# y00njaekim/CMU-11785-IDL-1.58bit-ASR

Hardware: AMD Instinct MI355X
Metric: mel-frames/sec (Conformer-S 1.58-bit train step) (higher is better)
Workload: dtype fp32; 1 GPU; conformer-s-1.58bit-train-step; global_batch=32, execution=hip-graph, per_gpu_batch=32, frames=1000, d_model=144, blocks=16, d_ff=576, heads=4, vocab=5004, parallelism=dp1, passes=teacher 2-bit + student 1-bit + SP, conv_pointwise=fp32 (reference)

## Files before the change

### cmu-11785-idl-1.58bit-asr_amd/csrc/convmod.hip

```cpp
#include <math.h>

#include <cstdlib>

#include "ob_fp.h"
#include "ob_launch.h"

namespace ob {

namespace {

constexpr int kThreads = 256;
constexpr size_t kMaxLds = 160 * 1024;

__device__ __forceinline__ float sigm(float x) { return fast_sigmoid(x); }
__device__ __forceinline__ float swish(float y) { return y * sigm(y); }

template <int KT, int R>
__device__ __forceinline__ void conv_window(const float* __restrict__ tile, int C, int c, int tl0,
                                            const float (&wt)[KT], float (&out)[R]) {
  float win[R + KT - 1];
#pragma unroll
  for (int i = 0; i < R + KT - 1; ++i) win[i] = tile[(tl0 + i) * C + c];
#pragma unroll
  for (int r = 0; r < R; ++r) {
// ... 342 lines not shown
}

__device__ __forceinline__ __amdgpu_buffer_rsrc_t rsrc(const float* base, size_t bytes) {
  return __builtin_amdgcn_make_buffer_rsrc(const_cast<float*>(base), (short)0, (int)bytes,
                                           0x00020000);
}
__device__ __forceinline__ float bload(__amdgpu_buffer_rsrc_t r, int off) {
  return __builtin_bit_cast(float, __builtin_amdgcn_raw_buffer_load_b32(r, off, 0, 0));
}
__device__ __forceinline__ void bstore(__amdgpu_buffer_rsrc_t r, int off, float v) {
  __builtin_amdgcn_raw_buffer_store_b32(__builtin_bit_cast(int, v), r, off, 0, 0);
}
typedef float cm_f32x4 __attribute__((ext_vector_type(4)));
__device__ __forceinline__ cm_f32x4 bload4(__amdgpu_buffer_rsrc_t r, int off) {
  return __builtin_bit_cast(cm_f32x4, __builtin_amdgcn_raw_buffer_load_b128(r, off, 0, 0));
}
constexpr int kLBQ = 4;

constexpr int kTT = 64;

template <int KT, int CG>
__global__ __launch_bounds__(kThreads) void cm_fwd_tile_kernel(
    const float* __restrict__ u, const float* __restrict__ wdw, const float* __restrict__ bdw,
    int T, int C, float* __restrict__ z, float* __restrict__ gout) {
  constexpr int P = KT / 2, W = kTT + KT - 1, NW = W * CG;
  constexpr int CQ = CG / 4, NQ = W * CQ;
  __shared__ __attribute__((aligned(16))) float gs[NW];
  const int t0 = blockIdx.x * kTT, b = blockIdx.y, c0 = blockIdx.z * CG;
  const size_t rb = (size_t)b * T;
  const __amdgpu_buffer_rsrc_t ru = rsrc(u + rb * 2 * C, (size_t)T * 2 * C * 4);
  for (int i0 = 0; i0 < NQ; i0 += kLBQ * kThreads) {
    cm_f32x4 va[kLBQ], vb[kLBQ];
#pragma unroll
    for (int q = 0; q < kLBQ; ++q) {
      const int i = i0 + threadIdx.x + q * kThreads;
      const int tl = i / CQ, cq = i - tl * CQ;
      const int t = t0 - P + tl;
      const int tc = t < 0 ? 0 : (t >= T ? T - 1 : t);
      const int off = 4 * (tc * 2 * C + c0 + 4 * (i < NQ ? cq : 0));
      va[q] = bload4(ru, off);
      vb[q] = bload4(ru, off + 4 * C);
    }
#pragma unroll
    for (int q = 0; q < kLBQ; ++q) {
      const int i = i0 + threadIdx.x + q * kThreads;
      if (i >= NQ) break;
      const int tl = i / CQ, cq = i - tl * CQ;
      const int t = t0 - P + tl;
      const bool in = t >= 0 && t < T;
      cm_f32x4 g4;
#pragma unroll
      for (int k = 0; k < 4; ++k) g4[k] = in ? va[q][k] * sigm(vb[q][k]) : 0.0f;
      *reinterpret_cast<cm_f32x4*>(gs + tl * CG + 4 * cq) = g4;
    }
  }
  __syncthreads();
  constexpr int nrb = kTT / kR;
  for (int it = threadIdx.x; it < CG * nrb; it += kThreads) {
    const int c = it % CG, tl0 = kR * (it / CG);
    if (t0 + tl0 >= T) break;
    float wt[KT], out[kR];
#pragma unroll
    for (int j = 0; j < KT; ++j) wt[j] = wdw[(c0 + c) * KT + j];
    conv_window<KT, kR>(gs, CG, c, tl0, wt, out);
    const float bc = bdw ? bdw[c0 + c] : 0.0f;
#pragma unroll
    for (int r = 0; r < kR; ++r) {
      const int t = t0 + tl0 + r;
      if (t < T) {
        z[(rb + t) * C + c0 + c] = out[r] + bc;
        gout[(rb + t) * C + c0 + c] = gs[(tl0 + r + P) * CG + c];
      }
    }
  }
}

template <int KT, int CG>
__global__ __launch_bounds__(kThreads) void cm_bwd_tile_kernel(
    const float* __restrict__ dv, const float* __restrict__ z, const float* __restrict__ g,
    const float* __restrict__ u, const float* __restrict__ stats, const float* __restrict__ coef,
    const float* __restrict__ gamma, const float* __restrict__ beta,
    const float* __restrict__ wdw, int64_t rows_pp, int T, int C, float* __restrict__ du,
    float* __restrict__ wpart, CmWgradEntry* __restrict__ tslot, CmWgradEntry ent) {
  constexpr int P = KT / 2, W = kTT + KT - 1, NW = W * CG;
  constexpr int CQ = CG / 4, NQ = W * CQ;
  if (tslot && blockIdx.x == 0 && blockIdx.y == 0 && blockIdx.z == 0 && threadIdx.x == 0) *tslot = ent;
  __shared__ __attribute__((aligned(16))) float dzs[NW];
  __shared__ __attribute__((aligned(16))) float gs[NW];
  const int t0 = blockIdx.x * kTT, b = blockIdx.y, c0 = blockIdx.z * CG;
  const size_t rb = (size_t)b * T;
  const int pass = (int)(rb / rows_pp);
  const size_t sl = (size_t)T * C * 4;
  const __amdgpu_buffer_rsrc_t rdv = rsrc(dv + rb * C, sl), rz = rsrc(z + rb * C, sl),
                               rg = rsrc(g + rb * C, sl);
  const __amdgpu_buffer_rsrc_t ru = rsrc(u + rb * 2 * C, 2 * sl), rdu = rsrc(du + rb * 2 * C, 2 * sl);
  for (int i0 = 0; i0 < NQ; i0 += kLBQ * kThreads) {
// ... 254 lines not shown
  cm_wgrad_final_block((int)blockIdx.x, wpart, nblk, C, K, dw, db);
}

__global__ __launch_bounds__(64 * kWfSlices) void cm_wgrad_table_kernel(
    const CmWgradEntry* __restrict__ tab) {
  const CmWgradEntry e = tab[blockIdx.y];
  if ((int)blockIdx.x * 64 >= e.C * (e.K + 1)) return;
  cm_wgrad_final_block((int)blockIdx.x, e.wpart, e.nblk, e.C, e.K, e.dw, e.db);
}

int rows_chunks(int64_t rows_pp, int64_t C) {
  const int64_t per = 8 * (kThreads / (C / 4));
  const int64_t s = (rows_pp + per - 1) / per;
  const int64_t cap = (rows_pp + kSB - 1) / kSB;
  const int64_t m = cap < 512 ? cap : 512;
  return (int)(s < 1 ? 1 : (s > m ? m : s));
}

int stats_chunks(int64_t rows_pp) {
  const int64_t s = (rows_pp + kSB - 1) / kSB;
  return (int)(s < 1 ? 1 : (s > 512 ? 512 : s));
}

size_t lds_fwd(int C, int K, int TT) { return sizeof(float) * ((size_t)(TT + K - 1) * C + (size_t)C * K); }
size_t lds_bwd(int C, int K, int TT) {
  return sizeof(float) * (2 * (size_t)(TT + K - 1) * C + (size_t)C * K);
}

int pick_tt(int64_t C, int64_t K) {
  for (int tt : {64, 32, 16})
    if (lds_bwd((int)C, (int)K, tt) <= kMaxLds) return tt;
  return 0;
}

}

int dw_threads(int64_t C, int64_t K) {
  int64_t n = C * ((K + 1 + 7) / 8);
  n = (n + 63) / 64 * 64;
  return (int)(n < 256 ? 256 : (n > 1024 ? 1024 : n));
}

bool convmod_supported(int64_t C, int64_t K) {
  return C >= 1 && K >= 1 && K % 2 == 1 && K <= 127 && pick_tt(C, K) > 0;
}

size_t convmod_workspace(int64_t P, int64_t Bt, int64_t T, int64_t C, int64_t K) {
  const int64_t rows_pp = Bt / P * T;
  const int S = stats_chunks(rows_pp);
  const int64_t ntt = ceil_div(T, pick_tt(C, K));
  size_t b = sizeof(double) * (size_t)(P * S * C * 2);
  b += sizeof(float) * (size_t)(P * C * 2);
  b += sizeof(float) * (size_t)(Bt * ntt * C * (K + 1));
  b += 2 * sizeof(float) * (size_t)(Bt * T * C);
  return b + 256;
}

void launch_convmod_fwd(const float* u, const float* wdw, const float* bdw, const float* gamma,
                        const float* beta, int64_t P, int64_t Bt, int64_t T, int64_t C, int64_t K,
                        float eps, float* z, float* g, float* stats, float* v, void* ws,
                        hipStream_t s) {
  const int64_t rows_pp = Bt / P * T;
  const int S = stats_chunks(rows_pp);
  double* part = reinterpret_cast<double*>(ws);
  const int TT = pick_tt(C, K);
  const dim3 gdw((unsigned)ceil_div(T, TT), (unsigned)Bt);
  const int cg = TT == kTT ? tile_cg(C, K) : 0;
  if (cg) {
    const dim3 gt((unsigned)ceil_div(T, kTT), (unsigned)Bt, (unsigned)(C / cg));
    if (cg == 48)
      hipLaunchKernelGGL((cm_fwd_tile_kernel<31, 48>), gt, dim3(kThreads), 0, s, u, wdw, bdw,
                         (int)T, (int)C, z, g);
    else if (cg == 32)
      hipLaunchKernelGGL((cm_fwd_tile_kernel<31, 32>), gt, dim3(kThreads), 0, s, u, wdw, bdw,
                         (int)T, (int)C, z, g);
    else
      hipLaunchKernelGGL((cm_fwd_tile_kernel<31, 16>), gt, dim3(kThreads), 0, s, u, wdw, bdw,
                         (int)T, (int)C, z, g);
  } else if (K == 31)
    hipLaunchKernelGGL(cm_glu_dw_fwd_kernel<31>, gdw, dim3(dw_threads(C, K)), lds_fwd((int)C, (int)K, TT),
                       s, u, wdw, bdw, (int)T, (int)C, (int)K, TT, z, g);
  else
    hipLaunchKernelGGL(cm_glu_dw_fwd_kernel<0>, gdw, dim3(dw_threads(C, K)), lds_fwd((int)C, (int)K, TT),
                       s, u, wdw, bdw, (int)T, (int)C, (int)K, TT, z, g);
  const bool rowvec = C % 4 == 0 && C / 4 <= kThreads && Bt * T < (1ll << 31);
  const int Sr = rowvec ? rows_chunks(rows_pp, C) : S;
  if (rowvec)
    hipLaunchKernelGGL(cm_sums_rows_kernel<0>, dim3((unsigned)Sr, (unsigned)P), dim3(kThreads), 0, s,
                       (const float*)z, (const float*)nullptr, (const float*)nullptr,
                       (const float*)nullptr, (const float*)nullptr, rows_pp, (int)C, Sr, part);
  else
    hipLaunchKernelGGL(cm_stats_part_kernel, dim3((unsigned)S, (unsigned)P), dim3(kThreads), 0, s,
                       (const float*)z, rows_pp, (int)C, S, part);
  hipLaunchKernelGGL(cm_stats_final_kernel, dim3((unsigned)(P * C)), dim3(64), 0, s,
                     (const double*)part, (int)P, (int)C, Sr, rows_pp, eps, stats);
  const int64_t total = Bt * T * C;
  int64_t blocks = ceil_div(total, kThreads);
  if (blocks > 8192) blocks = 8192;
  if (rowvec) {
    const int rl = kThreads / (int)(C / 4);
    const int64_t rb = ceil_div(Bt * T, rl);
    hipLaunchKernelGGL(cm_bn_swish_rows_kernel, dim3((unsigned)(rb < 8192 ? rb : 8192)),
                       dim3(kThreads), 0, s, (const float*)z, (const float*)stats, gamma, beta,
                       (int)rows_pp, (int)(Bt * T), (int)C, v);
  } else {
    hipLaunchKernelGGL(cm_bn_swish_fwd_kernel, dim3((unsigned)blocks), dim3(kThreads), 0, s,
                       (const float*)z, (const float*)stats, gamma, beta, rows_pp, (int)C, total, v);
  }
}

void launch_convmod_bwd(const float* dv, const float* u, const float* z, const float* g,
                        const float* stats, const float* wdw, const float* gamma,
                        const float* beta, int64_t P, int64_t Bt, int64_t T, int64_t C, int64_t K,
                        float* du, float* dwdw, float* dbdw, float* dgamma, float* dbeta, void* ws,
                        hipStream_t s, const CmDefer* defer) {
  const int64_t rows_pp = Bt / P * T;
  const int S = stats_chunks(rows_pp);
  const int TT = pick_tt(C, K);
  const int64_t ntt = ceil_div(T, TT);
  double* part = reinterpret_cast<double*>(ws);
  float* coef = reinterpret_cast<float*>(part + (size_t)(P * S * C * 2));
  float* wpart = coef + (size_t)(P * C * 2);
  float* dz = wpart + (size_t)(Bt * ntt * C * (K + 1));
  float* dg = dz + (size_t)(Bt * T * C);
  const int64_t total = Bt * T * C;
  int64_t eblocks = ceil_div(total, kThreads);
  if (eblocks > 8192) eblocks = 8192;
  const bool rowvec = C % 4 == 0 && C / 4 <= kThreads;
  const int Sr = rowvec ? rows_chunks(rows_pp, C) : S;
  if (rowvec)
    hipLaunchKernelGGL(cm_sums_rows_kernel<1>, dim3((unsigned)Sr, (unsigned)P), dim3(kThreads), 0, s,
                       z, dv, stats, gamma, beta, rows_pp, (int)C, Sr, part);
  else
    hipLaunchKernelGGL(cm_bn_bwd_part_kernel, dim3((unsigned)S, (unsigned)P), dim3(kThreads), 0, s,
                       dv, z, stats, gamma, beta, rows_pp, (int)C, S, part);
  hipLaunchKernelGGL(cm_bn_bwd_final_kernel, dim3((unsigned)C), dim3(64), 0, s,
                     (const double*)part, (int)P, (int)C, Sr, rows_pp, coef, dgamma, dbeta);
  const int cg = TT == kTT ? tile_cg(C, K) : 0;
  if (cg) {
    const dim3 gt((unsigned)ntt, (unsigned)Bt, (unsigned)(C / cg));
    const bool dfr = defer && defer->table && Bt * ntt > 0;
    CmWgradEntry* tslot = dfr ? defer->table + defer->slot : nullptr;
    const CmWgradEntry ent{wpart, dwdw, dbdw, (int)(Bt * ntt), (int)C, (int)K};
#define OB_CM_BWD_TILE(CG)                                                                      \
// ... 42 lines not shown
```

### cmu-11785-idl-1.58bit-asr_amd/csrc/tgemm.hip

```cpp
#include <cstdlib>

#include "ob_drop.h"
#include "ob_fp.h"
#include "ob_ln.h"
#include "ob_launch.h"
#include "ob_quant.h"

namespace ob {

namespace {

typedef float f32x4 __attribute__((ext_vector_type(4)));
typedef __bf16 bf16x8 __attribute__((ext_vector_type(8)));
typedef uint32_t u32x4 __attribute__((ext_vector_type(4)));

constexpr int kThreads = 256;
constexpr int kRows = 64;
constexpr size_t kMaxLds = 80 * 1024;
constexpr int kTargetBlocks = 512;
constexpr int kTargetBlocksLongK = 256;
constexpr int kByteWaves = 8;
constexpr int kBPad = 16;
constexpr int kBytePad = 8;

// ... 346 lines not shown
      }
      __builtin_amdgcn_sched_barrier(0);
      weight_image();
    } else {
      constexpr int kWpt = (16 * NT * 2 * NCH + kThr - 1) / kThr;
      uint32_t wv[kWpt];
#pragma unroll
      for (int i = 0; i < kWpt; ++i) wv[i] = word_at(threadIdx.x + i * kThr);
      if constexpr (kCross) {
        const float* a0 = arow_of(jof(it0 < itN ? it0 : rg));
#pragma unroll
        for (int c = 0; c < kWin; ++c) ldc(a0, c, buf[c][0], buf[c][1]);
      }
      __builtin_amdgcn_sched_barrier(0);
#pragma unroll
      for (int i = 0; i < kWpt; ++i) decode_store(threadIdx.x + i * kThr, wv[i]);
    }
  } else if (alpha_raw >= 2) {
    weight_image();
  } else {
    for (int idx = threadIdx.x; idx < nwords; idx += kThr) decode_store(idx, word_at(idx));
  }
  [[maybe_unused]] float* lnp = nullptr;
  if constexpr (EPI == kEpiResidual && BYTE && NT == 9 && MS == 1) {
    lnp = reinterpret_cast<float*>(smem + epi_stage_off(NT, kpad, BYTE) +
                                   (size_t)WV * 16 * (16 * NT + 4) * sizeof(float));
    if (ep.nln > 0 && threadIdx.x < 16 * NT) {
      const int c = threadIdx.x;
      lnp[c] = ep.lng[0] ? ep.lng[0][c] : 1.0f;
      lnp[16 * NT + c] = ep.lnb[0] ? ep.lnb[0][c] : 0.0f;
      lnp[32 * NT + c] = ep.nln > 1 && ep.lng[1] ? ep.lng[1][c] : 1.0f;
      lnp[48 * NT + c] = ep.nln > 1 && ep.lnb[1] ? ep.lnb[1][c] : 0.0f;
    }
  }
  __syncthreads();
  TG_STAMP(0);

  const __bf16* brow = bimg + r * stride + kg;
  const unsigned char* brow8 = reinterpret_cast<const unsigned char*>(smem) + r * stride + kg;
  const float a_eff = MS > 1 ? 2.0f
                      : BYTE ? 2.0f * effective_alpha(alpha, alpha_raw)
                             : effective_alpha(alpha, alpha_raw);
  const uint32_t dkey = (EPI != kEpiNone && ep.dc.on) ? drop_key(ep.rng[0], ep.rng[1] + ep.rng_off) : 0u;
  float bcol[NT];
#pragma unroll
  for (int t = 0; t < NT; ++t) {
    const int col = n0 + 16 * t + r;
    bcol[t] = (bias && col < N) ? bias[col] : 0.0f;
  }
// ... 131 lines not shown
            if (orow < M && cl < 16 * NT) {
              const f32x4 y = *reinterpret_cast<const f32x4*>(st + row * kLd + cl);
              o = epi_store4<EPI>(ep, dkey, C + orow * N + n0 + cl, rowbase + orow, n0 + cl, N, y,
                                  valid, rr[it & 1][i]);
            }
#pragma unroll
            for (int e = 0; e < 4; ++e) v[i][e] = o[e];
          }
          if (ep.nln > 0 && orow < M) {
            float v2[3][4] = {};
            lnrow::ln_row_v<3, 4>(v, lnp, lnp + 16 * NT, rowbase + orow, N, ep.lneps[0],
                                  ep.lny[0], ep.lnmean[0], ep.lnrstd[0], nullptr, 0.0f, &v2);
            if (ep.nln > 1)
              lnrow::ln_row_v<3, 4>(v2, lnp + 32 * NT, lnp + 48 * NT, rowbase + orow, N,
                                    ep.lneps[1], ep.lny[1], ep.lnmean[1], ep.lnrstd[1]);
          }
        }
        asm volatile("s_waitcnt lgkmcnt(0)" ::: "memory");
        __builtin_amdgcn_sched_barrier(0);
        TG_STAMP(2);
        continue;
      }
      constexpr bool kHasR = EPI == kEpiResidual || EPI == kEpiSwishDropBwd;
      bool rvalid[kEpiCW];
#pragma unroll
      for (int it = 0; it < kEpiCW; ++it) {
        rvalid[it] = true;
        if (EPI == kEpiResidual && ep.lens) {
          const int64_t grow = rowbase + m0 + (it * 64 + lane) / kQ;
          if (grow < ((int64_t)1 << 31)) {
            const uint32_t bb = (uint32_t)grow / (uint32_t)ep.T;
            rvalid[it] = (int)((uint32_t)grow - bb * (uint32_t)ep.T) < ep.lens[bb];
          } else {
            const int64_t bb = grow / ep.T;
            rvalid[it] = (grow - bb * ep.T) < ep.lens[bb];
          }
        }
      }
#pragma unroll
      for (int c0 = 0; c0 < NT; c0 += kEpiCW) {
        f32x4 rpre[kEpiCW];
        if constexpr (kHasR) {
#pragma unroll
          for (int it = 0; it < kEpiCW; ++it) {
            const int idx = it * 64 + lane, row = idx / kQ, c4 = idx - row * kQ;
            const int64_t orow = m0 + row < M ? m0 + row : M - 1;
            const int col = min(n0 + 16 * c0 + 4 * c4, N - 4);
            rpre[it] = *reinterpret_cast<const f32x4*>(ep.R + (rowbase + orow) * N + col);
          }
        }
#pragma unroll
        for (int t = 0; t < kEpiCW; ++t) {
          if (c0 + t >= NT) continue;
#pragma unroll
          for (int reg = 0; reg < 4; ++reg)
            stg[(4 * g + reg) * kEpiLd + 16 * t + r] = fmaf(a_eff, acc[c0 + t][reg], bcol[c0 + t]);
        }
        asm volatile("s_waitcnt lgkmcnt(0)" ::: "memory");
        __builtin_amdgcn_sched_barrier(0);
#pragma unroll
        for (int it = 0; it < kEpiCW; ++it) {
          const int idx = it * 64 + lane, row = idx / kQ, c4 = idx - row * kQ;
          const int64_t orow = m0 + row;
          const int col = n0 + 16 * c0 + 4 * c4;
          const f32x4 y = *reinterpret_cast<const f32x4*>(stg + row * kEpiLd + 4 * c4);
          if (orow < M && col < N && 4 * c4 < 16 * (NT - c0)) {
            if constexpr (EPI == kEpiNone) {
              *reinterpret_cast<f32x4*>(C + orow * N + col) = y;
              if (EPI == kEpiSwishDrop)
                *reinterpret_cast<f32x4*>(ep.C2 + (rowbase + orow) * N + col) = y;
            } else {
              epi_store4<EPI>(ep, dkey, C + orow * N + col, rowbase + orow, col, N, y, rvalid[it],
                              rpre[it]);
            }
          }
        }
        asm volatile("s_waitcnt lgkmcnt(0)" ::: "memory");
        __builtin_amdgcn_sched_barrier(0);
      }
      TG_STAMP(2);
      continue;
    }
    if constexpr (!VEC_EPI) {

    constexpr bool kHasR = EPI == kEpiResidual || EPI == kEpiSwishDropBwd;
    constexpr int kPre = 2;
    float rv[NT][4];
    auto load_r = [&](int t) {
      const int col = min(n0 + 16 * t + r, N - 1);
#pragma unroll
      for (int reg = 0; reg < 4; ++reg) {
        const int64_t orow = min(m0 + 4 * g + reg, M - 1);
        rv[t][reg] = ep.R[(rowbase + orow) * N + col];
      }
    };
    if constexpr (kHasR) {
#pragma unroll
      for (int t = 0; t < kPre && t < NT; ++t) load_r(t);
    }
#pragma unroll
    for (int t = 0; t < NT; ++t) {
// ... 128 lines not shown
      return nt;
  return 0;
}

template <int NT>
void launch_bf16x3(const float* A, int64_t M, int64_t K, const uint32_t* codes, int64_t N,
                   const float* alpha, int alpha_raw, const float* bias, float* C,
                   const uint32_t* codes1, const int* pass_bits, int P, const EpiArgs& ep,
                   hipStream_t s, bool byte = false) {
  const int n_ct = ep.glayers * (int)ceil_div(N, 16 * NT);
  const int n16 = (int)ceil_div(M, 16);
  const int wv = byte ? kByteWaves : 4;
  const int target = K > 256 ? kTargetBlocksLongK
                     : ep.mode == kEpiSwishDropBwd ? kTargetBlocks * 3 / 2
                                                   : kTargetBlocks;
  int rgroups = target / (n_ct * P);
  if (rgroups > ceil_div(n16, wv)) rgroups = (int)ceil_div(n16, wv);
  if (rgroups < 1) rgroups = 1;
  const dim3 grid((unsigned)(rgroups * n_ct), (unsigned)P);
  const int kpad = (int)((K + 31) & ~int64_t(31));
  const size_t lds = epi_stage_off(NT, kpad, byte) +
                     (byte && ep.mode == kEpiResidual
                          ? (size_t)wv * 16 * (16 * NT + 4) * sizeof(float) + 4 * 16 * NT * sizeof(float)
                          : epi_stage_bytes(NT, wv));
  const int KW = (int)ceil_div(K, 16);
  const bool vec = (N % 4 == 0) && aligned16(C) && (ep.mode != kEpiSwishDrop || aligned16(ep.C2)) &&
                   ((ep.mode != kEpiResidual && ep.mode != kEpiSwishDropBwd) || aligned16(ep.R));
#define OB_TGEMM_E(NCH, E)                                                                     \
  if (vec)                                                                                    \
    hipLaunchKernelGGL((tgemm_bf16x3_kernel<NT, NCH, E, true>), grid, dim3(kThreads), lds, s,  \
                       A, M, (int)K, codes, KW, (int)N, n_ct, n16, rgroups, alpha, alpha_raw,  \
                       bias, C, codes1, pass_bits, ep);                                         \
  else                                                                                        \
    hipLaunchKernelGGL((tgemm_bf16x3_kernel<NT, NCH, E, false>), grid, dim3(kThreads), lds, s, \
                       A, M, (int)K, codes, KW, (int)N, n_ct, n16, rgroups, alpha, alpha_raw,  \
                       bias, C, codes1, pass_bits, ep)
  if constexpr (NT == 9) {
    if (byte) {
#define OB_TGEMM_B(E)                                                                            \
  if (vec)                                                                                      \
    hipLaunchKernelGGL((tgemm_bf16x3_kernel<9, 18, E, true, true, 1, kByteWaves>), grid,         \
                       dim3(64 * kByteWaves), lds, s,                                            \
                       A, M, (int)K, codes, KW, (int)N, n_ct, n16, rgroups, alpha, alpha_raw,    \
                       bias, C, codes1, pass_bits, ep);                                           \
  else                                                                                          \
    hipLaunchKernelGGL((tgemm_bf16x3_kernel<9, 18, E, false, true, 1, kByteWaves>), grid,        \
                       dim3(64 * kByteWaves), lds,                                               \
// ... 107 lines not shown
    ep.galpha[i] = alpha[i];
    ep.gbias[i] = bias[i];
    ep.gC[i] = C[i];
  }
#define OB_NTG(V)                                                                                \
  case V:                                                                                        \
    launch_bf16x3<V>(A, M, K, codes[0], N, alpha[0], alpha_raw, bias[0], C[0], codes1[0],       \
                     pass_bits, P, ep, s);                                                       \
    return true;
  switch (nt) {
    OB_NTG(12)
    OB_NTG(9)
    OB_NTG(6)
    OB_NTG(4)
    OB_NTG(3)
    OB_NTG(2)
    OB_NTG(1)
    default: return false;
  }
#undef OB_NTG
}

bool ternary_residual_ln_supported(int64_t K, int64_t N, int alpha_raw) {
  return (K + 31) / 32 == 18 && K % 4 == 0 && N == 144 && alpha_raw < 2 && !use_f32_gemm() &&
         pick_nt(N, K, kEpiResidual) > 0;
}

bool launch_ternary_dx_sum(int G, const float* const* dY, int P, int64_t M, int64_t N,
                           const uint32_t* const* codes_t, const uint32_t* const* codes_t1,
                           const int* pass_bits, const float* const* alpha, int alpha_raw,
                           int64_t K, float* dX, hipStream_t s) {
  if (G != 3 || N != 144 || K <= 0 || K % 144 != 0 || alpha_raw >= 2 || use_f32_gemm())
    return false;
  for (int i = 0; i < G; ++i)
    if (!aligned16(dY[i])) return false;
  if (!aligned16(dX)) return false;
  if (M == 0 || P == 0) return true;
  EpiArgs ep{};
  ep.glayers = 1;
  ep.mode = kEpiNone;
  for (int i = 0; i < G; ++i) {
    ep.gA[i] = dY[i];
    ep.gcodes[i] = codes_t[i];
    ep.gcodes1[i] = codes_t1[i];
    ep.galpha[i] = alpha[i];
  }
  constexpr int kNch = 15;
  const int n_ct = (int)(K / 144);
// ... 28 lines not shown
```

### cmu-11785-idl-1.58bit-asr_amd/onebit_asr/conformer.py

```python
from __future__ import annotations

import math
from typing import List, Optional, Sequence

import torch
import torch.nn as nn
import torch.nn.functional as F

from .attention import fused_attention_supported, rel_pos_attention
from .conv import (conv2d_bias_relu, conv_module_fused, conv_module_supported, depthwise_conv1d,
                   subsample_convs, subsample_supported)
from .decattn import dec_attention, dec_attention_grouped, dec_attention_supported
from .embedding import embedding
from .fused import (ffn_residual, ffn_residual_i8, fused_supported, i8_fused_supported,
                    i8_linear, linear_residual, linear_residual_i8, qkv_projections)
from .layernorm import (Int8Act, fused_layernorm_supported, layer_norm, layer_norm_amax,
                        layer_norm_pair,
                        layer_norm_fork, layer_norm_i8)
from .linear import linear, linear_rows_split
from .quant import DeviceBits, PassBits, QuantizedLinear, StackedBits

__all__ = [
    "LayerNorm", "FeedForwardModule", "RelPositionalEncoding", "MHSA", "ConvModule",
    "Conv2dSubsampling", "ConformerBlock", "ConformerEncoder", "TransformerDecoder",
# ... 105 lines not shown

    def __init__(self, d_model: int, n_heads: int, dropout: float):
        super().__init__()
        assert d_model % n_heads == 0
        self.d_model = d_model
        self.n_heads = n_heads
        self.d_head = d_model // n_heads
        self.ln = LayerNorm(d_model)
        self.q_proj = QuantizedLinear(d_model, d_model)
        self.k_proj = QuantizedLinear(d_model, d_model)
        self.v_proj = QuantizedLinear(d_model, d_model)
        self.pos_proj = QuantizedLinear(d_model, d_model)
        self.out_proj = QuantizedLinear(d_model, d_model)
        self.dropout = nn.Dropout(dropout)
        self.pos_bias_u = nn.Parameter(torch.randn(self.n_heads, self.d_head) * 0.01)
        self.pos_bias_v = nn.Parameter(torch.randn(self.n_heads, self.d_head) * 0.01)

    def rel_shift(self, x):
        return rel_shift(x)

    def _heads(self, t: torch.Tensor, batch: int) -> torch.Tensor:
        return t.view(batch, -1, self.n_heads, self.d_head).transpose(1, 2)

    def _fused(self, x, h, mask, bitwidth, pos_emb):
        bsz, tlen, width = x.shape
        if isinstance(h, Int8Act):
            qp, kp, vp = (i8_linear(h, m, bitwidth) for m in (self.q_proj, self.k_proj, self.v_proj))
        elif fused_supported(h, self.q_proj, self.k_proj, self.v_proj, bitwidth=bitwidth):
            qp, kp, vp = qkv_projections(h, self.q_proj, self.k_proj, self.v_proj, bitwidth)
        else:
            qp = self.q_proj(h, bitwidth)
            kp = self.k_proj(h, bitwidth)
            vp = self.v_proj(h, bitwidth)
        if isinstance(bitwidth, PassBits):
            P = bitwidth.passes
            pe = getattr(pos_emb, "_ob_rows", None)
            if pe is None or pe.shape[0] != P * tlen:
                pe = pos_emb.expand(P, tlen, width).reshape(P * tlen, width)
                pos_emb._ob_rows = pe
            pp = self.pos_proj(pe, bitwidth).view(P, tlen, width)
        else:
            pp = self.pos_proj(pos_emb, bitwidth).view(1, tlen, width)
        if mask is None:
            lens = torch.full((bsz,), tlen, dtype=torch.int32, device=x.device)
        else:
            lens = getattr(mask, "_ob_lens", None)
            if lens is None:
                lens = mask[:, :, 0].sum(dim=1, dtype=torch.int32)
        p = self.dropout.p if self.training else 0.0
        ctx = rel_pos_attention(qp, kp, vp, pp, self.pos_bias_u, self.pos_bias_v, lens,
                                self.n_heads, p)
        if fused_supported(ctx, self.out_proj, bitwidth=bitwidth):
            return linear_residual(ctx, x, self.out_proj, bitwidth, p, 1.0,
                                   None if mask is None else lens, tlen)
        if i8_fused_supported(ctx, self.out_proj, bitwidth=bitwidth, p_drop=p):
            return linear_residual_i8(ctx, x, self.out_proj, bitwidth, 1.0,
                                      None if mask is None else lens, tlen)
        out = self.dropout(self.out_proj(ctx, bitwidth))
        return x + _pad_rows(out, mask)

    def forward(self, x, mask, bitwidth: int, pos_emb: torch.Tensor):
        bsz, tlen, width = x.shape
        assert width == self.d_model, f"Expected {self.d_model}, got {width}"
        if fused_attention_supported(x, self.d_head) and fused_supported(x, self.out_proj,
                                                                         bitwidth=bitwidth):
            h, xr = self.ln.fork(x)
            return self._fused(xr, h, mask, bitwidth, pos_emb)
        if (fused_attention_supported(x, self.d_head) and self.ln.emit_amax
                and fused_layernorm_supported(x, width)
                and i8_fused_supported(x, self.q_proj, self.k_proj, self.v_proj,
                                       bitwidth=bitwidth, p_drop=self.dropout.p if self.training else 0.0)):
            return self._fused(x, self.ln.forward_i8(x), mask, bitwidth, pos_emb)
        h = self.ln(x)
        if fused_attention_supported(h, self.d_head):
            return self._fused(x, h, mask, bitwidth, pos_emb)
        q = self._heads(self.q_proj(h, bitwidth), bsz)
        k = self._heads(self.k_proj(h, bitwidth), bsz)
        v = self._heads(self.v_proj(h, bitwidth), bsz)
        u_bias = self.pos_bias_u.view(1, self.n_heads, 1, self.d_head)
        v_bias = self.pos_bias_v.view(1, self.n_heads, 1, self.d_head)
        content = torch.matmul(q + u_bias, k.transpose(-2, -1))
        if isinstance(bitwidth, PassBits):
            P = bitwidth.passes
            pe = pos_emb.expand(P, tlen, width).reshape(P * tlen, width)
            p = self.pos_proj(pe, bitwidth).view(P, 1, tlen, self.n_heads, self.d_head)
            qv = (q + v_bias).view(P, bsz // P, self.n_heads, tlen, self.d_head)
            bd = torch.matmul(qv, p.permute(0, 1, 3, 4, 2))
            position = rel_shift(bd.view(bsz, self.n_heads, tlen, tlen))
        else:
            p = self._heads(self.pos_proj(pos_emb, bitwidth), 1)
# ... 88 lines not shown
        else:
            y = self.conv(x.unsqueeze(1))
        bsz, ch, tsub, fsub = y.shape
        y = y.transpose(1, 2).reshape(bsz, tsub, ch * fsub)
        return linear(y, self.out.weight, self.out.bias)


class ConformerBlock(nn.Module):

    def __init__(self, d_model: int, d_ff: int, n_heads: int, conv_kernel: int, dropout: float,
                 block_index: int, quantize_conv_pointwise: bool = False):
        super().__init__()
        self.block_index = block_index
        self.ff1 = FeedForwardModule(d_model, d_ff, dropout)
        self.mhsa = MHSA(d_model, n_heads, dropout)
        self.conv = ConvModule(d_model, kernel_size=conv_kernel, dropout=dropout,
                               quantize_pointwise=quantize_conv_pointwise)
        self.ff2 = FeedForwardModule(d_model, d_ff, dropout)
        self.ln = LayerNorm(d_model)

    def forward(self, x, src_mask, bitwidth_linear: int, pos_emb: torch.Tensor,
                next_ln: Optional["LayerNorm"] = None):
        x = self.ff1(x, bitwidth_linear, ln_next=[self.mhsa.ln])
        x = self.mhsa(x, src_mask, bitwidth_linear, pos_emb)
        passes = bitwidth_linear.passes if isinstance(bitwidth_linear, PassBits) else 1
        x = self.conv(x, passes=passes,
                      bitwidth=bitwidth_linear if self.conv.quantize_pointwise else None)
        x = self.ff2(x, bitwidth_linear,
                     ln_next=[self.ln] if next_ln is None or next_ln.emit_amax else [self.ln, next_ln])
        return self.ln(x) if next_ln is None else self.ln.pair(x, next_ln)


def block_bitwidths(n_layers: int, precision: int, sp_mask: Optional[Sequence[int]]) -> List[int]:
    if isinstance(sp_mask, (DeviceBits, StackedBits)):
        return [sp_mask[i] for i in range(n_layers)]
    out = []
    for i in range(n_layers):
        bw = precision if sp_mask is None else (1 if sp_mask[i] == 1 else 2)
        out.append(bw if bw in (1, 2) else 32)
    return out


class ConformerEncoder(nn.Module):
    def __init__(self, input_dim: int, d_model: int, n_layers: int, n_heads: int,
                 d_ff: int, conv_kernel: int, dropout: float,
                 quantize_conv_pointwise: bool = False):
        super().__init__()
# ... 268 lines not shown
```

### cmu-11785-idl-1.58bit-asr_amd/onebit_asr/fused.py

```python
from __future__ import annotations

import ctypes
import os
from typing import Dict, Optional

import torch

from . import _lib, deferred
from .layernorm import GradScale, Int8Act, attach_grad_scale
from .quant import PassBits, QuantizedLinear

__all__ = ["ffn_residual", "linear_residual", "fused_supported", "advance_step",
           "i8_fused_supported", "ffn_residual_i8", "linear_residual_i8", "qkv_projections",
           "i8_linear"]

_DW_GROUP = True
_DX_SUM = True
_QKV_FWD_GROUP = True
_STATE: Dict[torch.device, list] = {}


def _seed() -> int:
    return (int(torch.initial_seed()) * 0x9E3779B97F4A7C15 + 0x5851F42D) & ((1 << 62) - 1)

# ... 194 lines not shown
            _lib.check(lib.ob_drop_scale_bwd(gout.data_ptr(), rows, n2, 0.5, p, _lib.ptr(rng),
                                             off2, None, 0, dy2.data_ptr(), stream),
                       "ob_drop_scale_bwd")
        dpre = torch.empty((rows, n1), dtype=torch.float32, device=gout.device)
        _lib.check(lib.ob_bitlinear_bwd_dx_swish_drop(
            dy2.data_ptr(), P, m, n2, codes2[2].data_ptr(), codes2[3].data_ptr(), _lib.ptr(pb),
            a2.data_ptr(), codes2.dx_raw, n1, pre.data_ptr(), p, _lib.ptr(rng), off1,
            dpre.data_ptr(), stream),
            "ob_bitlinear_bwd_dx_swish_drop")
        gw2, ga2, gb2 = _dw(lib, dy2, act, P, m, n2, n1, w2, a2, ctx.has_bias[1], pb, bits, stream,
                            ctx.biases[1], codes2.dense)
        gh = _dx(lib, dpre, P, m, n1, codes1, pb, a1, k, stream) if ctx.needs_input_grad[0] else None
        gw1, ga1, gb1 = _dw(lib, dpre, h, P, m, n1, k, w1, a1, ctx.has_bias[0], pb, bits, stream,
                            ctx.biases[0], codes1.dense)
        return gh, gout, gw1, ga1, gb1, gw2, ga2, gb2, None, None


_LN_EPI = True


class _LinearResidualFn(torch.autograd.Function):

    @staticmethod
    def forward(ctx, x, resid, w, a, b, meta):
        P, pb, bits, codes, rscale, p, rng, off, lens, T, _ = meta
        rows, k = x.shape
        m = rows // P
        n = w.shape[0]
        lib = _lib.load()
        out = torch.empty((rows, n), dtype=torch.float32, device=x.device)
        _lib.check(lib.ob_bitlinear_fwd_residual(
            x.data_ptr(), P, m, k, codes[0].data_ptr(), codes[1].data_ptr(), _lib.ptr(pb),
            a.data_ptr(), codes.fwd_raw, _lib.ptr(b), n, resid.data_ptr(), rscale, p, _lib.ptr(rng), off,
            _lib.ptr(lens), T, out.data_ptr(), _lib.stream_of(x)), "ob_bitlinear_fwd_residual")
        ctx.meta = meta
        ctx.has_bias = b is not None
        ctx.bias = b
        deferred.note(w, a, b)
        ctx.save_for_backward(x, w, a)
        return out

    @staticmethod
    def backward(ctx, gout):
        x, w, a = ctx.saved_tensors
        P, pb, bits, codes, rscale, p, rng, off, lens, T, spec = ctx.meta
        gout = gout.contiguous()
        rows, k = x.shape
        m = rows // P
        n = w.shape[0]
        lib = _lib.load()
        stream = _lib.stream_of(gout)
        dy = spec.take(gout)
        if dy is None:
            dy = torch.empty_like(gout)
            _lib.check(lib.ob_drop_scale_bwd(gout.data_ptr(), rows, n, rscale, p, _lib.ptr(rng),
                                             off, _lib.ptr(lens), T, dy.data_ptr(), stream),
                       "ob_drop_scale_bwd")
        gx = _dx(lib, dy, P, m, n, codes, pb, a, k, stream) if ctx.needs_input_grad[0] else None
        gw, ga, gb = _dw(lib, dy, x, P, m, n, k, w, a, ctx.has_bias, pb, bits, stream, ctx.bias,
                         codes.dense)
        return gx, gout, gw, ga, gb, None


class _QKVFn(torch.autograd.Function):

    @staticmethod
    def forward(ctx, h, wq, aq, bq, wk, ak, bk, wv, av, bv, meta):
        P, pb, bits, codes = meta
        rows, k = h.shape
        m = rows // P
        lib = _lib.load()
        stream = _lib.stream_of(h)
        outs = []
        if pb is not None and _QKV_FWD_GROUP and wq.shape == wk.shape == wv.shape and \
                codes[0].fwd_raw == codes[1].fwd_raw == codes[2].fwd_raw:
            n = wq.shape[0]
            outs = [torch.empty((rows, n), dtype=torch.float32, device=h.device) for _ in range(3)]
            arrs = [_lib.ptr_array(v) for v in (
                [c[0].data_ptr() for c in codes], [c[1].data_ptr() for c in codes],
                [aq.data_ptr(), ak.data_ptr(), av.data_ptr()],
                [_lib.ptr(bq), _lib.ptr(bk), _lib.ptr(bv)], [y.data_ptr() for y in outs])]
            ad = [ctypes.addressof(x) for x in arrs]
            _lib.check(lib.ob_bitlinear_fwd_passes_group(
                3, h.data_ptr(), P, m, k, ad[0], ad[1], pb.data_ptr(), ad[2], codes[0].fwd_raw,
# ... 131 lines not shown
    if h2.shape[0] % P:
        raise ValueError(f"{h2.shape[0]} rows do not split into {P} passes")
    rng, off1 = _rng(h.device) if p_drop > 0 else (None, 0)
    off2 = _rng(h.device)[1] if p_drop > 0 else 0
    spec = GradScale(0.5, p_drop, rng, off2)
    meta = (P, pb, bits, _codes(lin1, P, bits), _codes(lin2, P, bits), float(p_drop), rng,
            off1, off2, spec)
    box = []
    lnreq = (([(w, b, float(e)) for w, b, e in ln_next], box)
             if ln_next and _LN_EPI and torch.is_grad_enabled() and 1 <= len(ln_next) <= 2
             else None)
    out = _FFNFn.apply(h2, x2, lin1.weight, lin1.alpha, lin1.bias, lin2.weight, lin2.alpha,
                       lin2.bias, meta, lnreq)
    out = attach_grad_scale(out.view(x.shape), spec)
    if box:
        out._ob_ln_pre = box[0]
        if len(box) > 1:
            out._ob_ln_pre2 = box[1]
    return out


def linear_residual(inp: torch.Tensor, x: torch.Tensor, lin: QuantizedLinear, bitwidth,
                    p_drop: float, rscale: float = 1.0, lens: Optional[torch.Tensor] = None,
                    frames: int = 0) -> torch.Tensor:
    P, pb, bits = _bits_args(bitwidth)
    i2, x2 = _flat(inp, lin.in_features), _flat(x, lin.out_features)
    if i2.shape[0] % P:
        raise ValueError(f"{i2.shape[0]} rows do not split into {P} passes")
    rng, off = _rng(inp.device) if p_drop > 0 else (None, 0)
    if lens is not None:
        lens = lens.to(torch.int32).contiguous()
    spec = GradScale(rscale, p_drop, rng, off, lens, frames)
    meta = (P, pb, bits, _codes(lin, P, bits), float(rscale), float(p_drop), rng, off, lens,
            int(frames), spec)
    out = _LinearResidualFn.apply(i2, x2, lin.weight, lin.alpha, lin.bias, meta)
    return attach_grad_scale(out.view(x.shape), spec)



def i8_fused_supported(x: torch.Tensor, *layers: QuantizedLinear, bitwidth=None,
                       p_drop: float = 0.0) -> bool:
    if os.environ.get("OB_FUSED", "1") == "0" or p_drop > 0.0 or torch.is_grad_enabled():
        return False
    if isinstance(bitwidth, PassBits) or bitwidth not in (1, 2):
        return False
    for m in layers:
        if m._packed is not None:
            m._check_packed_use(bitwidth)
    lib = _lib.load()
    return (x.is_cuda and x.dtype == torch.float32
            and all(m.act_quant == "absmax_int8" and m.quant_off is None
                    and m.out_features % 4 == 0 and m.in_features % 16 == 0
                    and m.in_features <= 576 for m in layers)
            and lib is not None)


def _i8_epi(a2: torch.Tensor, amax: torch.Tensor, lin: QuantizedLinear, bits: int, mode: int,
            R: Optional[torch.Tensor] = None, rscale: float = 1.0,
            lens: Optional[torch.Tensor] = None, frames: int = 0):
# ... 71 lines not shown
```

Baseline: 1.381 million mel-frames/s.

## Fuse conv-module BN stats into tiled forward and LayerNorm into attention out-proj epilogue

The tiled depthwise-conv forward kernel now accumulates per-channel sum and sum-of-squares in double while writing z, reduces them in LDS reused from the window buffer, and writes per-tile partials. The separate stats pass that re-read z is dropped and only the final reduction kernel remains. Separately, the attention out-projection residual GEMM gains a non-byte LayerNorm epilogue for N=144, so the conv module's pre-LayerNorm is produced from registers instead of by its own kernel. This adds register pressure and LDS to both kernels, and widens the set of residual-GEMM shapes allowed to take the LayerNorm path.

```diff
diff --git a/cmu-11785-idl-1.58bit-asr_amd/csrc/convmod.hip b/cmu-11785-idl-1.58bit-asr_amd/csrc/convmod.hip
--- a/cmu-11785-idl-1.58bit-asr_amd/csrc/convmod.hip
+++ b/cmu-11785-idl-1.58bit-asr_amd/csrc/convmod.hip
@@ -388,9 +388,13 @@
 template <int KT, int CG>
 __global__ __launch_bounds__(kThreads) void cm_fwd_tile_kernel(
     const float* __restrict__ u, const float* __restrict__ wdw, const float* __restrict__ bdw,
-    int T, int C, float* __restrict__ z, float* __restrict__ gout) {
+    int T, int C, float* __restrict__ z, float* __restrict__ gout, int Bp,
+    double* __restrict__ part) {
   constexpr int P = KT / 2, W = kTT + KT - 1, NW = W * CG;
   constexpr int CQ = CG / 4, NQ = W * CQ;
+  constexpr int NIT = (CG * (kTT / kR) + kThreads - 1) / kThreads;
+  static_assert(sizeof(float) * NW >= sizeof(double) * 2 * CG * (kTT / kR),
+                "the frame groups' sums reuse the window's LDS");
   __shared__ __attribute__((aligned(16))) float gs[NW];
   const int t0 = blockIdx.x * kTT, b = blockIdx.y, c0 = blockIdx.z * CG;
   const size_t rb = (size_t)b * T;
@@ -422,9 +426,14 @@
   }
   __syncthreads();
   constexpr int nrb = kTT / kR;
-  for (int it = threadIdx.x; it < CG * nrb; it += kThreads) {
+  double s1[NIT], s2[NIT];
+#pragma unroll
+  for (int k = 0; k < NIT; ++k) {
+    s1[k] = 0.0;
+    s2[k] = 0.0;
+    const int it = threadIdx.x + k * kThreads;
     const int c = it % CG, tl0 = kR * (it / CG);
-    if (t0 + tl0 >= T) break;
+    if (it >= CG * nrb || t0 + tl0 >= T) continue;
     float wt[KT], out[kR];
 #pragma unroll
     for (int j = 0; j < KT; ++j) wt[j] = wdw[(c0 + c) * KT + j];
@@ -434,10 +443,37 @@
     for (int r = 0; r < kR; ++r) {
       const int t = t0 + tl0 + r;
       if (t < T) {
-        z[(rb + t) * C + c0 + c] = out[r] + bc;
+        const float zv = out[r] + bc;
+        z[(rb + t) * C + c0 + c] = zv;
         gout[(rb + t) * C + c0 + c] = gs[(tl0 + r + P) * CG + c];
-      }
-    }
+        s1[k] += (double)zv;
+        s2[k] += (double)zv * zv;
+      }
+    }
+  }
+  __syncthreads();
+  double* red = reinterpret_cast<double*>(gs);
+#pragma unroll
+  for (int k = 0; k < NIT; ++k) {
+    const int it = threadIdx.x + k * kThreads;
+    if (it < CG * nrb) {
+      red[2 * it] = s1[k];
+      red[2 * it + 1] = s2[k];
+    }
+  }
+  __syncthreads();
+  const int p = b / Bp, ntile = (int)gridDim.x, S = Bp * ntile;
+  if (threadIdx.x < CG) {
+    double t1 = 0.0, t2 = 0.0;
+#pragma unroll
+    for (int q = 0; q < nrb; ++q) {
+      t1 += red[2 * (q * CG + threadIdx.x)];
+      t2 += red[2 * (q * CG + threadIdx.x) + 1];
+    }
+    const int chunk = (b - p * Bp) * ntile + (int)blockIdx.x;
+    double* o = part + (((size_t)p * C + c0 + threadIdx.x) * S + chunk) * 2;
+    o[0] = t1;
+    o[1] = t2;
   }
 }
 
@@ -738,6 +774,8 @@
   return (int)(s < 1 ? 1 : (s > 512 ? 512 : s));
 }
 
+int tile_chunks(int64_t Bp, int64_t T) { return (int)(Bp * ceil_div(T, kTT)); }
+
 size_t lds_fwd(int C, int K, int TT) { return sizeof(float) * ((size_t)(TT + K - 1) * C + (size_t)C * K); }
 size_t lds_bwd(int C, int K, int TT) {
   return sizeof(float) * (2 * (size_t)(TT + K - 1) * C + (size_t)C * K);
@@ -749,6 +787,14 @@
   return 0;
 }
 
+bool tiled(int64_t C, int64_t K) { return pick_tt(C, K) == kTT && tile_cg(C, K) > 0; }
+
+int part_chunks(int64_t P, int64_t Bt, int64_t T, int64_t C, int64_t K) {
+  const int S = stats_chunks(Bt / P * T);
+  const int St = tiled(C, K) ? tile_chunks(Bt / P, T) : 0;
+  return St > S ? St : S;
+}
+
 }
 
 int dw_threads(int64_t C, int64_t K) {
@@ -762,8 +808,7 @@
 }
 
 size_t convmod_workspace(int64_t P, int64_t Bt, int64_t T, int64_t C, int64_t K) {
-  const int64_t rows_pp = Bt / P * T;
-  const int S = stats_chunks(rows_pp);
+  const int64_t S = part_chunks(P, Bt, T, C, K);
   const int64_t ntt = ceil_div(T, pick_tt(C, K));
   size_t b = sizeof(double) * (size_t)(P * S * C * 2);
   b += sizeof(float) * (size_t)(P * C * 2);
@@ -781,35 +826,38 @@
   double* part = reinterpret_cast<double*>(ws);
   const int TT = pick_tt(C, K);
   const dim3 gdw((unsigned)ceil_div(T, TT), (unsigned)Bt);
-  const int cg = TT == kTT ? tile_cg(C, K) : 0;
+  const int cg = tiled(C, K) ? tile_cg(C, K) : 0;
+  const bool rowvec = C % 4 == 0 && C / 4 <= kThreads && Bt * T < (1ll << 31);
   if (cg) {
     const dim3 gt((unsigned)ceil_div(T, kTT), (unsigned)Bt, (unsigned)(C / cg));
-    if (cg == 48)
-      hipLaunchKernelGGL((cm_fwd_tile_kernel<31, 48>), gt, dim3(kThreads), 0, s, u, wdw, bdw,
-                         (int)T, (int)C, z, g);
-    else if (cg == 32)
-      hipLaunchKernelGGL((cm_fwd_tile_kernel<31, 32>), gt, dim3(kThreads), 0, s, u, wdw, bdw,
-                         (int)T, (int)C, z, g);
+#define OB_CM_FWD_TILE(CG)                                                                     \
+  hipLaunchKernelGGL((cm_fwd_tile_kernel<31, CG>), gt, dim3(kThreads), 0, s, u, wdw, bdw, (int)T, \
+                     (int)C, z, g, (int)(Bt / P), part)
+    if (cg == 48) OB_CM_FWD_TILE(48);
+    else if (cg == 32) OB_CM_FWD_TILE(32);
+    else OB_CM_FWD_TILE(16);
+#undef OB_CM_FWD_TILE
+    hipLaunchKernelGGL(cm_stats_final_kernel, dim3((unsigned)(P * C)), dim3(64), 0, s,
+                       (const double*)part, (int)P, (int)C, tile_chunks(Bt / P, T), rows_pp, eps,
+                       stats);
+  } else {
+    if (K == 31)
+      hipLaunchKernelGGL(cm_glu_dw_fwd_kernel<31>, gdw, dim3(dw_threads(C, K)),
+                         lds_fwd((int)C, (int)K, TT), s, u, wdw, bdw, (int)T, (int)C, (int)K, TT, z, g);
     else
-      hipLaunchKernelGGL((cm_fwd_tile_kernel<31, 16>), gt, dim3(kThreads), 0, s, u, wdw, bdw,
-                         (int)T, (int)C, z, g);
-  } else if (K == 31)
-    hipLaunchKernelGGL(cm_glu_dw_fwd_kernel<31>, gdw, dim3(dw_threads(C, K)), lds_fwd((int)C, (int)K, TT),
-                       s, u, wdw, bdw, (int)T, (int)C, (int)K, TT, z, g);
-  else
-    hipLaunchKernelGGL(cm_glu_dw_fwd_kernel<0>, gdw, dim3(dw_threads(C, K)), lds_fwd((int)C, (int)K, TT),
-                       s, u, wdw, bdw, (int)T, (int)C, (int)K, TT, z, g);
-  const bool rowvec = C % 4 == 0 && C / 4 <= kThreads && Bt * T < (1ll << 31);
-  const int Sr = rowvec ? rows_chunks(rows_pp, C) : S;
-  if (rowvec)
-    hipLaunchKernelGGL(cm_sums_rows_kernel<0>, dim3((unsigned)Sr, (unsigned)P), dim3(kThreads), 0, s,
-                       (const float*)z, (const float*)nullptr, (const float*)nullptr,
-                       (const float*)nullptr, (const float*)nullptr, rows_pp, (int)C, Sr, part);
-  else
-    hipLaunchKernelGGL(cm_stats_part_kernel, dim3((unsigned)S, (unsigned)P), dim3(kThreads), 0, s,
-                       (const float*)z, rows_pp, (int)C, S, part);
-  hipLaunchKernelGGL(cm_stats_final_kernel, dim3((unsigned)(P * C)), dim3(64), 0, s,
-                     (const double*)part, (int)P, (int)C, Sr, rows_pp, eps, stats);
+      hipLaunchKernelGGL(cm_glu_dw_fwd_kernel<0>, gdw, dim3(dw_threads(C, K)),
+                         lds_fwd((int)C, (int)K, TT), s, u, wdw, bdw, (int)T, (int)C, (int)K, TT, z, g);
+    const int Sr = rowvec ? rows_chunks(rows_pp, C) : S;
+    if (rowvec)
+      hipLaunchKernelGGL(cm_sums_rows_kernel<0>, dim3((unsigned)Sr, (unsigned)P), dim3(kThreads), 0,
+                         s, (const float*)z, (const float*)nullptr, (const float*)nullptr,
+                         (const float*)nullptr, (const float*)nullptr, rows_pp, (int)C, Sr, part);
+    else
+      hipLaunchKernelGGL(cm_stats_part_kernel, dim3((unsigned)S, (unsigned)P), dim3(kThreads), 0, s,
+                         (const float*)z, rows_pp, (int)C, S, part);
+    hipLaunchKernelGGL(cm_stats_final_kernel, dim3((unsigned)(P * C)), dim3(64), 0, s,
+                       (const double*)part, (int)P, (int)C, Sr, rows_pp, eps, stats);
+  }
   const int64_t total = Bt * T * C;
   int64_t blocks = ceil_div(total, kThreads);
   if (blocks > 8192) blocks = 8192;
@@ -835,7 +883,7 @@
   const int TT = pick_tt(C, K);
   const int64_t ntt = ceil_div(T, TT);
   double* part = reinterpret_cast<double*>(ws);
-  float* coef = reinterpret_cast<float*>(part + (size_t)(P * S * C * 2));
+  float* coef = reinterpret_cast<float*>(part + (size_t)(P * part_chunks(P, Bt, T, C, K) * C * 2));
   float* wpart = coef + (size_t)(P * C * 2);
   float* dz = wpart + (size_t)(Bt * ntt * C * (K + 1));
   float* dg = dz + (size_t)(Bt * T * C);
diff --git a/cmu-11785-idl-1.58bit-asr_amd/csrc/tgemm.hip b/cmu-11785-idl-1.58bit-asr_amd/csrc/tgemm.hip
--- a/cmu-11785-idl-1.58bit-asr_amd/csrc/tgemm.hip
+++ b/cmu-11785-idl-1.58bit-asr_amd/csrc/tgemm.hip
@@ -392,9 +392,10 @@
     for (int idx = threadIdx.x; idx < nwords; idx += kThr) decode_store(idx, word_at(idx));
   }
   [[maybe_unused]] float* lnp = nullptr;
-  if constexpr (EPI == kEpiResidual && BYTE && NT == 9 && MS == 1) {
+  if constexpr (EPI == kEpiResidual && NT == 9 && MS == 1) {
     lnp = reinterpret_cast<float*>(smem + epi_stage_off(NT, kpad, BYTE) +
-                                   (size_t)WV * 16 * (16 * NT + 4) * sizeof(float));
+                                   (BYTE ? (size_t)WV * 16 * (16 * NT + 4) * sizeof(float)
+                                         : epi_stage_bytes(NT, WV)));
     if (ep.nln > 0 && threadIdx.x < 16 * NT) {
       const int c = threadIdx.x;
       lnp[c] = ep.lng[0] ? ep.lng[0][c] : 1.0f;
@@ -572,6 +573,8 @@
         continue;
       }
       constexpr bool kHasR = EPI == kEpiResidual || EPI == kEpiSwishDropBwd;
+      constexpr bool kLnReg = EPI == kEpiResidual && !BYTE && NT == 9 && MS == 1;
+      [[maybe_unused]] float lnv[kLnReg ? kEpiCW : 1][3][4];
       bool rvalid[kEpiCW];
 #pragma unroll
       for (int it = 0; it < kEpiCW; ++it) {
@@ -614,19 +617,40 @@
           const int64_t orow = m0 + row;
           const int col = n0 + 16 * c0 + 4 * c4;
           const f32x4 y = *reinterpret_cast<const f32x4*>(stg + row * kEpiLd + 4 * c4);
+          [[maybe_unused]] f32x4 o = f32x4{0.f, 0.f, 0.f, 0.f};
           if (orow < M && col < N && 4 * c4 < 16 * (NT - c0)) {
             if constexpr (EPI == kEpiNone) {
               *reinterpret_cast<f32x4*>(C + orow * N + col) = y;
               if (EPI == kEpiSwishDrop)
                 *reinterpret_cast<f32x4*>(ep.C2 + (rowbase + orow) * N + col) = y;
             } else {
-              epi_store4<EPI>(ep, dkey, C + orow * N + col, rowbase + orow, col, N, y, rvalid[it],
-                              rpre[it]);
+              o = epi_store4<EPI>(ep, dkey, C + orow * N + col, rowbase + orow, col, N, y,
+                                  rvalid[it], rpre[it]);
             }
+          }
+          if constexpr (kLnReg) {
+#pragma unroll
+            for (int e = 0; e < 4; ++e) lnv[it][c0 / kEpiCW][e] = o[e];
           }
         }
         asm volatile("s_waitcnt lgkmcnt(0)" ::: "memory");
         __builtin_amdgcn_sched_barrier(0);
+      }
+      if constexpr (kLnReg) {
+        if (ep.nln > 0) {
+#pragma unroll
+          for (int it = 0; it < kEpiCW; ++it) {
+            const int64_t orow = m0 + it * 4 + (lane >> 4);
+            if (orow < M) {
+              float v2[3][4] = {};
+              lnrow::ln_row_v<3, 4>(lnv[it], lnp, lnp + 16 * NT, rowbase + orow, N, ep.lneps[0],
+                                    ep.lny[0], ep.lnmean[0], ep.lnrstd[0], nullptr, 0.0f, &v2);
+              if (ep.nln > 1)
+                lnrow::ln_row_v<3, 4>(v2, lnp + 32 * NT, lnp + 48 * NT, rowbase + orow, N,
+                                      ep.lneps[1], ep.lny[1], ep.lnmean[1], ep.lnrstd[1]);
+            }
+          }
+        }
       }
       TG_STAMP(2);
       continue;
@@ -801,7 +825,8 @@
   const size_t lds = epi_stage_off(NT, kpad, byte) +
                      (byte && ep.mode == kEpiResidual
                           ? (size_t)wv * 16 * (16 * NT + 4) * sizeof(float) + 4 * 16 * NT * sizeof(float)
-                          : epi_stage_bytes(NT, wv));
+                          : epi_stage_bytes(NT, wv) +
+                                (NT == 9 && ep.mode == kEpiResidual ? 4 * 16 * NT * sizeof(float) : 0));
   const int KW = (int)ceil_div(K, 16);
   const bool vec = (N % 4 == 0) && aligned16(C) && (ep.mode != kEpiSwishDrop || aligned16(ep.C2)) &&
                    ((ep.mode != kEpiResidual && ep.mode != kEpiSwishDropBwd) || aligned16(ep.R));
@@ -955,8 +980,10 @@
 }
 
 bool ternary_residual_ln_supported(int64_t K, int64_t N, int alpha_raw) {
-  return (K + 31) / 32 == 18 && K % 4 == 0 && N == 144 && alpha_raw < 2 && !use_f32_gemm() &&
-         pick_nt(N, K, kEpiResidual) > 0;
+  if (K % 4 != 0 || N != 144 || use_f32_gemm()) return false;
+  if ((K + 31) / 32 == 18 && alpha_raw < 2 && pick_nt(N, K, kEpiResidual) > 0)
+    return true;
+  return pick_nt(N, K, kEpiResidual) == 9;
 }
 
 bool launch_ternary_dx_sum(int G, const float* const* dY, int P, int64_t M, int64_t N,
diff --git a/cmu-11785-idl-1.58bit-asr_amd/onebit_asr/conformer.py b/cmu-11785-idl-1.58bit-asr_amd/onebit_asr/conformer.py
--- a/cmu-11785-idl-1.58bit-asr_amd/onebit_asr/conformer.py
+++ b/cmu-11785-idl-1.58bit-asr_amd/onebit_asr/conformer.py
@@ -151,7 +151,7 @@
     def _heads(self, t: torch.Tensor, batch: int) -> torch.Tensor:
         return t.view(batch, -1, self.n_heads, self.d_head).transpose(1, 2)
 
-    def _fused(self, x, h, mask, bitwidth, pos_emb):
+    def _fused(self, x, h, mask, bitwidth, pos_emb, ln_next=None):
         bsz, tlen, width = x.shape
         if isinstance(h, Int8Act):
             qp, kp, vp = (i8_linear(h, m, bitwidth) for m in (self.q_proj, self.k_proj, self.v_proj))
@@ -180,21 +180,24 @@
         ctx = rel_pos_attention(qp, kp, vp, pp, self.pos_bias_u, self.pos_bias_v, lens,
                                 self.n_heads, p)
         if fused_supported(ctx, self.out_proj, bitwidth=bitwidth):
+            lnn = ([(ln_next.ln.weight, ln_next.ln.bias, ln_next.ln.eps)]
+                   if ln_next is not None and not ln_next.emit_amax else None)
             return linear_residual(ctx, x, self.out_proj, bitwidth, p, 1.0,
-                                   None if mask is None else lens, tlen)
+                                   None if mask is None else lens, tlen, lnn)
         if i8_fused_supported(ctx, self.out_proj, bitwidth=bitwidth, p_drop=p):
             return linear_residual_i8(ctx, x, self.out_proj, bitwidth, 1.0,
                                       None if mask is None else lens, tlen)
         out = self.dropout(self.out_proj(ctx, bitwidth))
         return x + _pad_rows(out, mask)
 
-    def forward(self, x, mask, bitwidth: int, pos_emb: torch.Tensor):
+    def forward(self, x, mask, bitwidth: int, pos_emb: torch.Tensor,
+                ln_next: Optional["LayerNorm"] = None):
         bsz, tlen, width = x.shape
         assert width == self.d_model, f"Expected {self.d_model}, got {width}"
         if fused_attention_supported(x, self.d_head) and fused_supported(x, self.out_proj,
                                                                          bitwidth=bitwidth):
             h, xr = self.ln.fork(x)
-            return self._fused(xr, h, mask, bitwidth, pos_emb)
+            return self._fused(xr, h, mask, bitwidth, pos_emb, ln_next)
         if (fused_attention_supported(x, self.d_head) and self.ln.emit_amax
                 and fused_layernorm_supported(x, width)
                 and i8_fused_supported(x, self.q_proj, self.k_proj, self.v_proj,
@@ -329,7 +332,7 @@
     def forward(self, x, src_mask, bitwidth_linear: int, pos_emb: torch.Tensor,
                 next_ln: Optional["LayerNorm"] = None):
         x = self.ff1(x, bitwidth_linear, ln_next=[self.mhsa.ln])
-        x = self.mhsa(x, src_mask, bitwidth_linear, pos_emb)
+        x = self.mhsa(x, src_mask, bitwidth_linear, pos_emb, ln_next=self.conv.ln)
         passes = bitwidth_linear.passes if isinstance(bitwidth_linear, PassBits) else 1
         x = self.conv(x, passes=passes,
                       bitwidth=bitwidth_linear if self.conv.quantize_pointwise else None)
diff --git a/cmu-11785-idl-1.58bit-asr_amd/onebit_asr/fused.py b/cmu-11785-idl-1.58bit-asr_amd/onebit_asr/fused.py
--- a/cmu-11785-idl-1.58bit-asr_amd/onebit_asr/fused.py
+++ b/cmu-11785-idl-1.58bit-asr_amd/onebit_asr/fused.py
@@ -240,17 +240,34 @@
 class _LinearResidualFn(torch.autograd.Function):
 
     @staticmethod
-    def forward(ctx, x, resid, w, a, b, meta):
+    def forward(ctx, x, resid, w, a, b, meta, lnreq=None):
         P, pb, bits, codes, rscale, p, rng, off, lens, T, _ = meta
         rows, k = x.shape
         m = rows // P
         n = w.shape[0]
         lib = _lib.load()
         out = torch.empty((rows, n), dtype=torch.float32, device=x.device)
-        _lib.check(lib.ob_bitlinear_fwd_residual(
-            x.data_ptr(), P, m, k, codes[0].data_ptr(), codes[1].data_ptr(), _lib.ptr(pb),
-            a.data_ptr(), codes.fwd_raw, _lib.ptr(b), n, resid.data_ptr(), rscale, p, _lib.ptr(rng), off,
-            _lib.ptr(lens), T, out.data_ptr(), _lib.stream_of(x)), "ob_bitlinear_fwd_residual")
+        st = _lib.OB_ERR_SHAPE
+        if lnreq is not None:
+            (req,), box = lnreq
+            lno = (torch.empty_like(out), torch.empty((rows,), dtype=torch.float32, device=x.device),
+                   torch.empty((rows,), dtype=torch.float32, device=x.device))
+            st = lib.ob_bitlinear_fwd_residual_ln(
+                x.data_ptr(), P, m, k, codes[0].data_ptr(), codes[1].data_ptr(), _lib.ptr(pb),
+                a.data_ptr(), codes.fwd_raw, _lib.ptr(b), n, resid.data_ptr(), rscale, p,
+                _lib.ptr(rng), off, _lib.ptr(lens), T, out.data_ptr(), 1, _lib.ptr(req[0]),
+                _lib.ptr(req[1]), float(req[2]), *(t.data_ptr() for t in lno), None, None, 0.0,
+                None, None, None, _lib.stream_of(x))
+            if st == _lib.OB_OK:
+                box.append((*req, *lno))
+            elif st != _lib.OB_ERR_SHAPE:
+                _lib.check(st, "ob_bitlinear_fwd_residual_ln")
+        if st != _lib.OB_OK:
+            _lib.check(lib.ob_bitlinear_fwd_residual(
+                x.data_ptr(), P, m, k, codes[0].data_ptr(), codes[1].data_ptr(), _lib.ptr(pb),
+                a.data_ptr(), codes.fwd_raw, _lib.ptr(b), n, resid.data_ptr(), rscale, p,
+                _lib.ptr(rng), off, _lib.ptr(lens), T, out.data_ptr(), _lib.stream_of(x)),
+                "ob_bitlinear_fwd_residual")
         ctx.meta = meta
         ctx.has_bias = b is not None
         ctx.bias = b
@@ -277,7 +294,7 @@
         gx = _dx(lib, dy, P, m, n, codes, pb, a, k, stream) if ctx.needs_input_grad[0] else None
         gw, ga, gb = _dw(lib, dy, x, P, m, n, k, w, a, ctx.has_bias, pb, bits, stream, ctx.bias,
                          codes.dense)
-        return gx, gout, gw, ga, gb, None
+        return gx, gout, gw, ga, gb, None, None
 
 
 class _QKVFn(torch.autograd.Function):
@@ -455,7 +472,7 @@
 
 def linear_residual(inp: torch.Tensor, x: torch.Tensor, lin: QuantizedLinear, bitwidth,
                     p_drop: float, rscale: float = 1.0, lens: Optional[torch.Tensor] = None,
-                    frames: int = 0) -> torch.Tensor:
+                    frames: int = 0, ln_next=None) -> torch.Tensor:
     P, pb, bits = _bits_args(bitwidth)
     i2, x2 = _flat(inp, lin.in_features), _flat(x, lin.out_features)
     if i2.shape[0] % P:
@@ -466,8 +483,14 @@
     spec = GradScale(rscale, p_drop, rng, off, lens, frames)
     meta = (P, pb, bits, _codes(lin, P, bits), float(rscale), float(p_drop), rng, off, lens,
             int(frames), spec)
-    out = _LinearResidualFn.apply(i2, x2, lin.weight, lin.alpha, lin.bias, meta)
-    return attach_grad_scale(out.view(x.shape), spec)
+    box = []
+    lnreq = (([(w, b, float(e)) for w, b, e in ln_next], box)
+             if ln_next and _LN_EPI and torch.is_grad_enabled() and len(ln_next) == 1 else None)
+    out = _LinearResidualFn.apply(i2, x2, lin.weight, lin.alpha, lin.bias, meta, lnreq)
+    out = attach_grad_scale(out.view(x.shape), spec)
+    if box:
+        out._ob_ln_pre = box[0]
+    return out
 
 
 
```

New measurement: 1.390 million mel-frames/s, median of 6. No clear change (+0.7%).
